# minyoungpark1/Speech-Enhancement

Hardware: AMD Instinct MI355X
Metric: utterances/sec (2 s @16 kHz) CMGAN train step (higher is better)
Workload: dtype f32 (f16x3 split); 1 GPU; cmgan generator+discriminator train step (main_gan.py train_gan loop body), batch 16/GPU, 2 s @ 16 kHz, n_fft=400 hop=100, AdamW lr 5e-4, PESQ labels supplied, kaiming-init weights; fp32 results throughout: conv and token GEMMs as scaled fp16 hi/lo splits (3 MFMAs per product, 2^-24 relative, fp32 accumulate), attention on the same scaled fp16 splits (scales from measured operand maxima), everythi; global_batch=16, parallelism=dp1

## Files before the change

### include/se_hip.h

```cpp
#ifndef SE_HIP_H
#define SE_HIP_H
#include <stddef.h>
#include <stdint.h>

#ifdef __cplusplus
extern "C" {
#endif

#define SE_MAX_TAPS 16

enum { SE_PRO_NONE = 0, SE_PRO_LN = 1, SE_PRO_SWISH = 2, SE_PRO_AFFINE_SWISH = 3,
       SE_PRO_SWISH_DROP = 4,
       SE_PRO_DROP = 5,
       SE_PRO_GATE = 6 };
enum {
  SE_EPI_BIAS = 1,
  SE_EPI_ACCUM = 2,
  SE_EPI_RESID = 4,
  SE_EPI_GLU = 8,
  SE_EPI_STATS = 16,
  SE_EPI_SWISH_GRAD = 32,
  SE_EPI_SHUFFLE2 = 64,
  SE_EPI_DROP = 128,
  SE_EPI_GLU_GATE = 2048,
// ... 118 lines not shown
                          const float* dR2, float* dX, float* dg, float* db, long M, int C, float* amax_out, void* stream);
int se_col_stats(const float* X, int ld, int x_off, double* stats, int B, long P, int C, void* stream);
int se_norm_finalize(const double* stats, const float* g, const float* beta, float* mr, float* ss,
                     int nb, int C, double count, float eps, float* running_mean, float* running_var,
                     float momentum, void* stream);
int se_bn_eval_scale(const float* rm, const float* rv, const float* g, const float* beta, float* ss,
                     float* mr, int C, float eps, void* stream);
int se_affine_prelu(const float* X, int ldx, int x_off, const float* ss, const float* slope, float* Y,
                    int ldy, int y_off, int B, long P, int C, void* stream);
int se_inorm_prelu_fwd(const float* X, int ldx, int x_off, const double* stats, const float* g, const float* beta,
                       const float* slope, float* Y, int ldy, int y_off, float* mr, int B, long P, int C, double count,
                       float eps, void* stream);
int se_inorm_prelu_fwd_amax(const float* X, int ldx, int x_off, const double* stats, const float* g, const float* beta,
                       const float* slope, float* Y, int ldy, int y_off, float* mr, int B, long P, int C, double count,
                       float eps, float* amax_out, void* stream);
int se_norm_prelu_bwd(const float* X, int ldx, int x_off, const float* mr, const float* g,
                      const float* beta, const float* slope, const float* dY, int ldy, int y_off,
                      double* red, float* dX, int lddx, int dx_off, float* dg, float* dbeta,
                      float* dslope, int B, long P, int C, int per_batch, int act, int phase, double count,
                      void* stream);
int se_norm_prelu_bwd_amax(const float* X, int ldx, int x_off, const float* mr, const float* g,
                           const float* beta, const float* slope, const float* dY, int ldy, int y_off,
                           double* red, float* dX, int lddx, int dx_off, float* dg, float* dbeta,
                           float* dslope, int B, long P, int C, int per_batch, int act, int phase, double count,
                           float* amax_out, void* stream);

int se_attn_fwd(const float* QKV, const float* E, float* O, float* LSE, int nseq, int n, int inner,
                long outer_stride, long inner_stride, long pos_stride, int maxpos, float scale, void* stream);
int se_attn_fwd_es(const float* QKV, const float* E, const void* Es, long es_plane, float* O, float* LSE, int nseq, int n,
                   int inner, long outer_stride, long inner_stride, long pos_stride, int maxpos, float scale, void* stream);
int se_attn_bwd(const float* QKV, const float* E, const float* O, const float* dO, const float* LSE,
                float* dQKV, float* dE, int nseq, int n, int inner, long outer_stride,
                long inner_stride, long pos_stride, long ntok, int maxpos, float scale, void* ws, size_t ws_bytes,
                void* stream);

int se_attn_fwd_f16(const float* QKV, const void* Es, long es_plane, const float* qkv_amax, const float* e_amax, float* O,
                    float* LSE, int nseq, int n, int inner, long outer_stride, long inner_stride, long pos_stride, int maxpos,
                    float scale, void* stream);
int se_attn_bwd_f16_phase(const float* QKV, const float* E, const float* O, const float* dO, const float* LSE,
                          const float* delta, const float* qkv_amax, const float* do_amax, float* dqkv_amax, float* dQKV, float* dE,
                          int nseq, int n, int inner, long outer_stride, long inner_stride, long pos_stride, long ntok, int maxpos,
                          float scale, void* ws, size_t ws_bytes, int phase, void* stream);

int se_dwconv31(const float* X, const float* W, const float* bias, float* Y, double* stats, int flip,
                int nseq, int n, int inner, long outer_stride, long inner_stride, long pos_stride, void* stream);
int se_dwconv31_glu_bwd(const float* dH, const float* W, const float* U, const float* G, float* dZ, float* amax_out, int nseq,
                        int n, int inner, long outer_stride, long inner_stride, long pos_stride, void* stream);
size_t se_dwconv31_wgrad_workspace_bytes(void);
int se_dwconv31_bwd_fused(const float* dH, const float* W, const float* U, const float* G, float* dZ, float* amax_out, float* dW,
                          float* dbias, float* ws, long ntok, int nseq, int n, int inner, long outer_stride, long inner_stride,
                          long pos_stride, void* stream);
int se_dwconv31_wgrad(const float* X, const float* dY, float* dW, float* dbias, int nseq, int n, int inner,
                      long outer_stride, long inner_stride, long pos_stride, float* ws, void* stream);

int se_clip_scale(const float* x, float* c, int B, int L, void* stream);
int se_reflect_pad_scale(const float* x, const float* c, float* xp, int B, int L, int pad, void* stream);
int se_reflect_pad_bwd(const float* dxp, const float* c, float* dx, int B, int L, int pad, void* stream);
int se_compress_planes(const float* R, int ldr, float* P, long rows, int F, int comp, float pre_scale, void* stream);
int se_compress_planes_bwd(const float* R, int ldr, const float* dP, float* dR, long rows, int F, int comp,
                           float pre_scale, void* stream);
int se_uncompress_rows(const float* P, float* A, int lda, long rows, int F, int comp, float post_scale, void* stream);
int se_uncompress_rows_bwd(const float* P, const float* dA, int lda, float* dP, long rows, int F, int comp,
                           float post_scale, void* stream);
int se_stft_fused(const float* x, const float* c, const float* Wf, float* P, int B, int L, int n_fft, int hop, int comp,
                  float pre_scale, void* stream);
int se_istft_fused(const float* P, const float* Wi, const float* env, float* y, int B, int T, int n_fft, int hop, int comp,
                   float post_scale, void* stream);
int se_ola(const float* Fr, const float* env, float* y, int B, int T, int n_fft, int hop, int trim, int L, void* stream);
int se_ola_bwd(const float* dy, const float* env, float* dFr, int B, int T, int n_fft, int hop, void* stream);
int se_assemble(const float* mask, int ldm, const float* nin, const float* cplx, float* est, long n, void* stream);
int se_assemble_bwd(const float* est, const float* dest, const float* nin, float* dmask, int ldm, float* dcplx,
                    long n, void* stream);
int se_mask_tail(const float* U, int ldu, const float* wb, const float* slope, float* M, long n, int F, void* stream);
int se_mask_tail_bwd(const float* U, int ldu, const float* wb, const float* slope, const float* dM, float* dU,
                     double* dwb, float* dslope, long n, int F, void* stream);
int se_glu_bwd(const float* Z, const float* dU, float* dZ, long M, int H, void* stream);
int se_glu_bwd_amax(const float* Z, const float* dU, float* dZ, long M, int H, float* amax_out, void* stream);
int se_glu_bwd_gate(const float* U, const float* G, const float* dU, float* dZ, long M, int H, float* amax_out, void* stream);
int se_gate_tanh(const float* Y, float* G, long M, int C, void* stream);
int se_gate_tanh_bwd(const float* Y, const float* dG, float* dY, long M, int C, void* stream);
int se_spec_loss(const float* A, const float* Bp, double* sums, long n, void* stream);
int se_spec_loss_bwd(const float* A, const float* Bp, float* dA, const float* up, float cmag, float cri, long n,
                     int accumulate, void* stream);
int se_l1_loss(const float* a, long lda, const float* b, long ldb, double* sums, long rows, int L, void* stream);
int se_l1_loss_bwd(const float* a, long lda, const float* b, long ldb, float* da, const float* up, float ck,
                   long rows, int L, void* stream);
int se_adamw(float* p, const float* g, float* m, float* v, long n, float lr, float b1, float b2, float eps,
             float wd, int step, void* stream);
int se_sgd_nesterov(float* p, const float* g, float* buf, long n, float lr, float momentum, int first, void* stream);
int se_dot(const float* a, const float* b, double* out, long n, void* stream);
int se_grad_clip(float* g, long n, const double* sums, int nsum, float max_norm, void* stream);
int se_lars_step(float* p, const float* g, float* mu, const long* seg_off, int nseg, long max_seg, double* norms,
                 int adapt, float lr, float wd, float momentum, float trust_coef, void* stream);
int se_lamb_step(float* p, const float* g, float* m, float* v, const long* seg_off, int nseg, long max_seg,
                 double* norms, const double* gsum, int nsum, float max_grad_norm, int adapt, int trust_clip, float lr,
                 float wd, float b1, float b2, float beta3, float eps, float bc1, float bc2, void* stream);
int se_axpbypcz(const float* a, const float* b, const float* c, float* y, float alpha, float beta, float gamma,
                long n, void* stream);

int se_spectral_norm(int n, const float* const* W, float* const* u, float* const* v, float* const* Wn, const int* h,
                     const int* w, float* sigma, int train, float eps, void* stream);
int se_spectral_norm_bwd(int n, const float* const* dWn, const float* const* Wn, const float* const* u,
                         const float* const* v, const float* sigma, float* const* dW, const int* h, const int* w, void* stream);
size_t se_disc_tail_workspace_bytes(int B);
int se_disc_tail_fwd(const float* A, int B, int P, const float* W1, const float* b1, const float* mask, const float* slope1,
                     const float* W2, const float* b2, const float* sslope, float beta, float* out, float* ws, void* stream);
// ... 38 lines not shown
```

### speech-enhancement_amd/csrc/se_dwconv.hip

```cpp
#include <type_traits>
#include "se_common.h"

struct SeqGeom {
  int nseq, n, inner;
  long outer_stride, inner_stride, pos_stride;
};
static __device__ __forceinline__ long tok_of(const SeqGeom& g, int s, int p) {
  return (long)(s / g.inner) * g.outer_stride + (long)(s % g.inner) * g.inner_stride + (long)p * g.pos_stride;
}

constexpr int DW_C = 128, DW_K = 31;
#ifdef SE_DW_NT
#define DW_STORE(p, v) __builtin_nontemporal_store((v), (p))
#else
#define DW_STORE(p, v) (*(p) = (v))
#endif
#define DW_LOAD4(p) (*reinterpret_cast<const f32x4*>(p))

struct DwArgs {
  SeqGeom g;
  const float* X; const float* W; const float* bias; float* Y; double* stats; int flip;
  const float* Z; float* amax_out; const float* U;
};

// ... 222 lines not shown
        if (i < NR) {
#pragma unroll
          for (int o = 0; o < PPS; ++o) {
            const int k = i - o;
            if (k >= 0 && k < DW_K) acc[k] = __builtin_elementwise_fma(dy[o], xg[g & 1][j], acc[k]);
          }
        }
      }
    }
  }
  float* red = xs;
  float* prow = a.part + (long)blockIdx.x * 32 * DW_C;
#pragma unroll
  for (int k0 = 0; k0 < 32; k0 += 8) {
    __syncthreads();
#pragma unroll
    for (int kk = 0; kk < 8; ++kk) {
      const int k = k0 + kk;
      const f32x2 v = k < DW_K ? acc[k < DW_K ? k : 0] : bacc;
      *reinterpret_cast<f32x2*>(&red[((ps * 8 + kk) * DW_C) + cl * 2]) = v;
    }
    __syncthreads();
    for (int i = tid; i < 8 * DW_C; i += 512) {
      int kk = i >> 7, ch = i & 127;
      float t = 0.f;
#pragma unroll
      for (int sl = 0; sl < 8; ++sl) t += red[(sl * 8 + kk) * DW_C + ch];
      prow[(k0 + kk) * DW_C + ch] = t;
    }
  }
}

__global__ void dwconv_wgrad_reduce_kernel(const float* __restrict__ part, int nwg, float* __restrict__ dW,
                                           float* __restrict__ dbias) {
  const int i = blockIdx.x * blockDim.x + threadIdx.x;
  const int per = (nwg + gridDim.y - 1) / gridDim.y, w0 = blockIdx.y * per, w1 = w0 + per < nwg ? w0 + per : nwg;
  if (i >= 32 * DW_C || w0 >= w1) return;
  float v[16];
#pragma unroll
  for (int j = 0; j < 16; ++j) v[j] = w0 + j < w1 ? part[(long)(w0 + j) * 32 * DW_C + i] : 0.f;
  float t = 0.f;
#pragma unroll
  for (int j = 0; j < 16; ++j) t += v[j];
  for (int w = w0 + 16; w < w1; ++w) t += part[(long)w * 32 * DW_C + i];
  const int k = i >> 7, ch = i & 127;
  if (k < DW_K) atomicAdd(&dW[ch * DW_K + k], t);
  else if (dbias) atomicAdd(&dbias[ch], t);
}

struct DwBwdArgs {
  SeqGeom g;
  const float* dH; const float* W; const float* U; const float* Z; float* dZ; float* amax_out; float* part;
  unsigned bytes128, bytes256;
};
constexpr int FB_PPS = 7, FB_TILE = 16 * FB_PPS, FB_ROWS = FB_TILE + DW_K - 1, FB_NLD = (FB_ROWS * 32 + 1023) / 1024,
              FB_NLU = (FB_TILE * 32 + 1023) / 1024;
typedef unsigned u32x2fb_ __attribute__((ext_vector_type(2)));
#ifndef FB_NT
#define FB_NT 8
#endif
constexpr int FB_LDS_BYTES = (FB_ROWS * DW_C + FB_TILE * DW_C + DW_K * DW_C) * 4;

__global__ __launch_bounds__(1024) void dwconv_bwd_fused_kernel(DwBwdArgs a) {
  extern __shared__ __attribute__((aligned(16))) float fb_smem[];
  float* xs = fb_smem;
  float* us = fb_smem + FB_ROWS * DW_C;
  float* wt = us + FB_TILE * DW_C;
  const int tid = threadIdx.x, cl = tid & 63, ps = __builtin_amdgcn_readfirstlane(tid >> 6);
  const unsigned cl8 = (unsigned)cl * 8u;
  const int n = a.g.n;
  for (int i = tid; i < DW_C * DW_K; i += 1024) {
    const int ch = i / DW_K, k = i - ch * DW_K;
    wt[(DW_K - 1 - k) * DW_C + ch] = a.W[i];
  }
  const __amdgpu_buffer_rsrc_t rH = make_rsrc_(a.dH, a.bytes128), rU = make_rsrc_(a.U, a.bytes128), rG = make_rsrc_(a.Z, a.bytes128),
                               rD = make_rsrc_(a.dZ, a.bytes256);
  const int tiles = (n + FB_TILE - 1) / FB_TILE;
  const long nitems = (long)a.g.nseq * tiles;
  const int xcd = blockIdx.x & 7, slot = blockIdx.x >> 3, S = gridDim.x >> 3;
  const long Q = (nitems + 7) >> 3, ibase = (long)xcd * Q, iend = ibase + Q < nitems ? ibase + Q : nitems;
  const unsigned rsb = (unsigned)(a.g.pos_stride * DW_C * 4);
  float zmax = 0.f;
  float4 ld[FB_NLD], lu[FB_NLU];
  const int lrow = tid >> 5;
  const unsigned lane_off = (unsigned)lrow * rsb + (unsigned)(tid & 31) * 16u;
  auto request_rows = [&](long it) {
    const bool live = it < iend;
    const long itc = live ? it : 0;
    const int seq = (int)(itc / tiles), p0 = (int)(itc - (long)seq * tiles) * FB_TILE;
    const unsigned base = (unsigned)(((long)(seq / a.g.inner) * a.g.outer_stride + (long)(seq % a.g.inner) * a.g.inner_stride) * (DW_C * 4));
    const int plo = 15 - p0 > 0 ? 15 - p0 : 0;
    const int phi = n - (p0 - 15) < FB_ROWS ? n - (p0 - 15) : FB_ROWS;
    const unsigned span = live && phi > plo ? (unsigned)(phi - plo) : 0u;
    const unsigned uspan = live ? (unsigned)(n - p0 < FB_TILE ? n - p0 : FB_TILE) : 0u;
#pragma unroll
    for (int k = 0; k < FB_NLD; ++k) {
      const int row = lrow + 32 * k;
      const unsigned off = base + (unsigned)(p0 - 15 + 32 * k) * rsb + lane_off;
      ld[k] = buf_load4_(rH, (unsigned)(row - plo) < span ? off : BUF_OOB_);
    }
#pragma unroll
    for (int k = 0; k < FB_NLU; ++k) {
      const int row = lrow + 32 * k;
      const unsigned off = base + (unsigned)(p0 + 32 * k) * rsb + lane_off;
      lu[k] = buf_load4_(rU, (unsigned)row < uspan ? off : BUF_OOB_);
    }
  };
  constexpr int NT = FB_NT, NGRP = 32 / NT, NPART = 16 / NGRP, PLEN = FB_TILE / NPART;
  const int tg = ps % NGRP, ph = ps / NGRP;
  f32x2 wacc[NT];
#pragma unroll
  for (int j = 0; j < NT; ++j) wacc[j] = (f32x2){0.f, 0.f};
  request_rows(ibase + slot);
  for (long it = ibase + slot; it < iend; it += S) {
    const int seq = (int)(it / tiles), p0 = (int)(it - (long)seq * tiles) * FB_TILE;
    const unsigned base = (unsigned)(((long)(seq / a.g.inner) * a.g.outer_stride + (long)(seq % a.g.inner) * a.g.inner_stride) * (DW_C * 4));
    __syncthreads();
#pragma unroll
    for (int k = 0; k < FB_NLD; ++k) {
      const int row = lrow + 32 * k;
      if (row < FB_ROWS) *reinterpret_cast<float4*>(&xs[row * DW_C + (tid & 31) * 4]) = ld[k];
    }
#pragma unroll
    for (int k = 0; k < FB_NLU; ++k) {
      const int row = lrow + 32 * k;
      if (row < FB_TILE) *reinterpret_cast<float4*>(&us[row * DW_C + (tid & 31) * 4]) = lu[k];
    }
    __syncthreads();
    const int pbase = p0 + ps * FB_PPS;
    f32x2 gt[FB_PPS];
#pragma unroll
    for (int o = 0; o < FB_PPS; ++o)
      gt[o] = __builtin_bit_cast(f32x2, buf_load2_(rG, pbase + o < n ? base + (unsigned)(pbase + o) * rsb + cl8 : BUF_OOB_));
    {
      constexpr int NR = FB_PPS + DW_K - 1;
      const float* xrow = &xs[(ps * FB_PPS) * DW_C + cl * 2];
      f32x2 acc[FB_PPS];
#pragma unroll
      for (int o = 0; o < FB_PPS; ++o) acc[o] = (f32x2){0.f, 0.f};
#pragma unroll
      for (int h = 0; h < 2; ++h) {
        constexpr int KH = 16;
        const int K0 = h * KH, K1 = h == 0 ? KH : DW_K;
        f32x2 w[KH];
#pragma unroll
        for (int k = 0; k < KH; ++k)
          if (K0 + k < K1) w[k] = *reinterpret_cast<const f32x2*>(&wt[(K0 + k) * DW_C + cl * 2]);
        const int R0 = K0, R1 = K1 - 1 + FB_PPS;
        constexpr int GA = 4;
        f32x2 xg[2][GA];
#pragma unroll
        for (int j = 0; j < GA; ++j) xg[0][j] = *reinterpret_cast<const f32x2*>(xrow + (R0 + j) * DW_C);
#pragma unroll
        for (int g = 0; g < (KH + FB_PPS - 1 + GA - 1) / GA; ++g) {
          asm volatile("" ::: "memory");
          if (R0 + (g + 1) * GA < R1) {
#pragma unroll
            for (int j = 0; j < GA; ++j)
              if (R0 + (g + 1) * GA + j < R1) xg[(g + 1) & 1][j] = *reinterpret_cast<const f32x2*>(xrow + (R0 + (g + 1) * GA + j) * DW_C);
          }
          asm volatile("" ::: "memory");
#pragma unroll
          for (int j = 0; j < GA; ++j) {
            const int i = R0 + g * GA + j;
            if (i < R1) {
#pragma unroll
              for (int o = 0; o < FB_PPS; ++o) {
                const int k = i - o;
                if (k >= K0 && k < K1) acc[o] = __builtin_elementwise_fma(xg[g & 1][j], w[k - K0], acc[o]);
              }
            }
          }
        }
      }
#pragma unroll
      for (int o = 0; o < FB_PPS; ++o) asm volatile("" : "+v"(acc[o]));
      const float* urow = &us[(ps * FB_PPS) * DW_C + cl * 2];
#pragma unroll
      for (int o = 0; o < FB_PPS; ++o) {
// ... 29 lines not shown
        constexpr int UB = 2, BOFF = 17 - NT;
        static_assert(PLEN % UB == 0, "position part not a multiple of the read group");
        f32x2 r[NT];
#pragma unroll
        for (int jj = 1; jj < NT; ++jj)
          if (!(BIAS && jj == NT - 1)) r[jj] = *reinterpret_cast<const f32x2*>(xp - jj * DW_C);
#pragma unroll 1
        for (int qq = 0; qq < PLEN; qq += UB) {
          f32x2 uu[UB], r0[UB], rb[UB];
#pragma unroll
          for (int e = 0; e < UB; ++e) {
            uu[e] = *reinterpret_cast<const f32x2*>(up + (qq + e) * DW_C);
            r0[e] = *reinterpret_cast<const f32x2*>(xp + (qq + e) * DW_C);
            if constexpr (BIAS) rb[e] = *reinterpret_cast<const f32x2*>(xp + (qq + e + BOFF) * DW_C);
          }
#pragma unroll
          for (int e = 0; e < UB; ++e) {
            r[0] = r0[e];
#pragma unroll
            for (int jj = 0; jj < NT; ++jj) {
              if (BIAS && jj == NT - 1) wacc[jj] += rb[e];
              else wacc[jj] = __builtin_elementwise_fma(uu[e], r[jj], wacc[jj]);
            }
#pragma unroll
            for (int jj = NT - 1; jj >= 1; --jj) r[jj] = r[jj - 1];
          }
        }
      };
      if (tg == NGRP - 1) phase_b(std::true_type{}); else phase_b(std::false_type{});
    }
#endif
  }
  if (a.amax_out) {
    zmax = wave_max(zmax);
    if ((tid & 63) == 0) amax_raise_(a.amax_out, zmax);
  }
  __syncthreads();
  float* red = xs;
  int t2 = threadIdx.x;
  asm volatile("" : "+v"(t2));
  const int w2 = t2 >> 6, c2 = t2 & 63;
#pragma unroll
  for (int j = 0; j < NT; ++j) *reinterpret_cast<f32x2*>(&red[((w2 / NGRP) * 32 + NT * (w2 % NGRP) + j) * DW_C + c2 * 2]) = wacc[j];
  __syncthreads();
  float* prow = a.part + (long)blockIdx.x * 32 * DW_C;
  float4 t = *reinterpret_cast<const float4*>(red + t2 * 4);
#pragma unroll
  for (int h = 1; h < NPART; ++h) {
    const float4 v = *reinterpret_cast<const float4*>(red + h * 32 * DW_C + t2 * 4);
    t = make_float4(t.x + v.x, t.y + v.y, t.z + v.z, t.w + v.w);
  }
  *reinterpret_cast<float4*>(prow + t2 * 4) = t;
}

extern "C" int se_dwconv31(const float* X, const float* W, const float* bias, float* Y, double* stats, int flip,
                           int nseq, int n, int inner, long outer_stride, long inner_stride, long pos_stride,
                           void* stream) {
  SE_REQUIRE(X && W && Y && nseq > 0 && n > 0 && inner > 0, "dwconv31: bad arguments");
  SE_REQUIRE(pos_stride > 0 && pos_stride * DW_C * 160L < (1L << 30), "dwconv31: position stride too large for 32-bit tile offsets");
  DwArgs a{{nseq, n, inner, outer_stride, inner_stride, pos_stride}, X, W, bias, Y, stats, flip, nullptr, nullptr};
  const int pps = n <= 64 ? 8 : (n <= 104 ? 13 : 14);
  const long nitems = (long)nseq * cdiv(n, 8 * pps);
  const int nblk = nitems < 512 ? (int)((nitems + 7) / 8 * 8) : 512;
#ifdef SE_DW_TWIN
  if (pps == 13) hipLaunchKernelGGL((dwconv_kernel<13, false, true>), dim3(nblk), dim3(512), 0, as_stream(stream), a);
  else if (pps == 14) hipLaunchKernelGGL((dwconv_kernel<14, false, true>), dim3(nblk), dim3(512), 0, as_stream(stream), a);
  else
#endif
  if (pps == 8) hipLaunchKernelGGL(dwconv_kernel<8>, dim3(nblk), dim3(512), 0, as_stream(stream), a);
  else if (pps == 13) hipLaunchKernelGGL(dwconv_kernel<13>, dim3(nblk), dim3(512), 0, as_stream(stream), a);
  else hipLaunchKernelGGL(dwconv_kernel<14>, dim3(nblk), dim3(512), 0, as_stream(stream), a);
  return se_check_launch("se_dwconv31");
}

extern "C" int se_dwconv31_glu_bwd(const float* dH, const float* W, const float* U, const float* G, float* dZ, float* amax_out,
                                   int nseq, int n, int inner, long outer_stride, long inner_stride, long pos_stride,
                                   void* stream) {
  SE_REQUIRE(dH && W && U && G && dZ && nseq > 0 && n > 0 && inner > 0, "dwconv31_glu_bwd: bad arguments");
  SE_REQUIRE(pos_stride > 0 && pos_stride * DW_C * 320L < (1L << 30), "dwconv31_glu_bwd: position stride too large for 32-bit tile offsets");
  DwArgs a{{nseq, n, inner, outer_stride, inner_stride, pos_stride}, dH, W, nullptr, dZ, nullptr, 1, G, amax_out, U};
  const int pps = n <= 64 ? 8 : (n <= 104 ? 13 : 14);
  const long nitems = (long)nseq * cdiv(n, 8 * pps);
  const int nblk = nitems < 512 ? (int)((nitems + 7) / 8 * 8) : 512;
#ifdef SE_DW_TWIN
  if (pps == 13) hipLaunchKernelGGL((dwconv_kernel<13, true, true>), dim3(nblk), dim3(512), 0, as_stream(stream), a);
  else if (pps == 14) hipLaunchKernelGGL((dwconv_kernel<14, true, true>), dim3(nblk), dim3(512), 0, as_stream(stream), a);
  else
#endif
  if (pps == 8) hipLaunchKernelGGL((dwconv_kernel<8, true>), dim3(nblk), dim3(512), 0, as_stream(stream), a);
  else if (pps == 13) hipLaunchKernelGGL((dwconv_kernel<13, true>), dim3(nblk), dim3(512), 0, as_stream(stream), a);
  else hipLaunchKernelGGL((dwconv_kernel<14, true>), dim3(nblk), dim3(512), 0, as_stream(stream), a);
  return se_check_launch("se_dwconv31_glu_bwd");
}

extern "C" size_t se_dwconv31_wgrad_workspace_bytes(void) { return (size_t)512 * 32 * DW_C * sizeof(float); }

extern "C" int se_dwconv31_wgrad(const float* X, const float* dY, float* dW, float* dbias, int nseq, int n,
                                 int inner, long outer_stride, long inner_stride, long pos_stride, float* ws,
                                 void* stream) {
  SE_REQUIRE(X && dY && dW && ws && nseq > 0 && n > 0 && inner > 0, "dwconv31_wgrad: bad arguments");
  SE_REQUIRE(pos_stride > 0 && pos_stride * DW_C * 160L < (1L << 30), "dwconv31_wgrad: position stride too large for 32-bit tile offsets");
  DwWgradArgs a{{nseq, n, inner, outer_stride, inner_stride, pos_stride}, X, dY, dW, dbias, ws};
  const int pps = n <= 64 ? 8 : (n <= 104 ? 13 : 14);
  const long nitems = (long)nseq * cdiv(n, 8 * pps);
  const int nblk = nitems < 512 ? (int)((nitems + 7) / 8 * 8) : 512;
  if (pps == 8) hipLaunchKernelGGL(dwconv_wgrad_kernel<8>, dim3(nblk), dim3(512), 0, as_stream(stream), a);
  else if (pps == 13) hipLaunchKernelGGL(dwconv_wgrad_kernel<13>, dim3(nblk), dim3(512), 0, as_stream(stream), a);
  else hipLaunchKernelGGL(dwconv_wgrad_kernel<14>, dim3(nblk), dim3(512), 0, as_stream(stream), a);
  hipLaunchKernelGGL(dwconv_wgrad_reduce_kernel, dim3(32 * DW_C / 256, 32), dim3(256), 0, as_stream(stream), (const float*)ws, nblk,
                     dW, dbias);
  return se_check_launch("se_dwconv31_wgrad");
}

extern "C" int se_dwconv31_bwd_fused(const float* dH, const float* W, const float* U, const float* G, float* dZ, float* amax_out,
                                     float* dW, float* dbias, float* ws, long ntok, int nseq, int n, int inner, long outer_stride,
                                     long inner_stride, long pos_stride, void* stream) {
  SE_REQUIRE(dH && W && U && G && dZ && dW && ws && nseq > 0 && n > 0 && inner > 0 && ntok > 0, "dwconv31_bwd_fused: bad arguments");
  SE_REQUIRE(ntok * (DW_C * 8L) < (1L << 32) - 4096, "dwconv31_bwd_fused: operands beyond 32-bit buffer offsets (%ld tokens)", ntok);
  SE_REQUIRE(pos_stride > 0 && (long)(nseq - 1) / inner * outer_stride + (long)(inner - 1) * inner_stride + (long)(n - 1) * pos_stride < ntok,
             "dwconv31_bwd_fused: sequence geometry reaches past %ld tokens", ntok);
  DwBwdArgs a{{nseq, n, inner, outer_stride, inner_stride, pos_stride}, dH, W, U, G, dZ, amax_out, ws,
              (unsigned)(ntok * DW_C * 4), (unsigned)(ntok * DW_C * 8)};
  const long nitems = (long)nseq * cdiv(n, FB_TILE);
  const int ncu = se_cu_count();
  int nblk = nitems < ncu ? (int)((nitems + 7) / 8 * 8) : ncu / 8 * 8;
  if (nblk > 512) nblk = 512;
  static unsigned lds_done = 0;
  SE_REQUIRE(se_raise_lds((const void*)dwconv_bwd_fused_kernel, FB_LDS_BYTES, &lds_done), "dwconv31_bwd_fused: cannot raise the LDS limit");
  hipLaunchKernelGGL(dwconv_bwd_fused_kernel, dim3(nblk), dim3(1024), FB_LDS_BYTES, as_stream(stream), a);
  hipLaunchKernelGGL(dwconv_wgrad_reduce_kernel, dim3(32 * DW_C / 256, 32), dim3(256), 0, as_stream(stream), (const float*)ws, nblk,
                     dW, dbias);
  return se_check_launch("se_dwconv31_bwd_fused");
}
```

### speech-enhancement_amd/layers.py

```python
import ctypes as C

import torch

from . import _lib as L
from . import attention as A
from . import gemm as GM
from . import ops as O

EPS = 1e-5

import os as _os
EPS = 1e-5

import os as _os
_PREC = {'f32': 0, 'bf16x3': 1, 'bf16x6': 2, 'f16x3': 3}
CONV_PRECISION = _PREC[_os.environ.get('SE_CONV_PRECISION', 'f16x3')]
ACT_SEXP = 4
PW2_F16 = True
ATTN_O_SEXP = 4
ATTN_PRECISION = [_os.environ.get('SE_ATTN_PRECISION', 'f16x3')]


WGRAD_PRECISION = [_PREC[_os.environ.get('SE_WGRAD_PRECISION', 'f16x3')]]


FUSE_LN_BWD = True
FUSE_ROWSTATS = True
FUSE_GLU_BWD = True


def set_conv_precision(name, wgrad=None):
    global CONV_PRECISION
    CONV_PRECISION = _PREC[name]
    WGRAD_PRECISION[0] = _PREC[wgrad or name]


def _conv3_shape(taps, sf, C_in, Fo=None):
    if sf != 1 or C_in < 32 or len(taps) % 3 or (Fo is not None and Fo < 2):
        return False
    for i in range(0, len(taps), 3):
        if {t[0] for t in taps[i:i + 3]} != {taps[i][0]} or sorted(abs(t[1]) for t in taps[i:i + 3]) != [0, 1, 1] or \
                {t[1] for t in taps[i:i + 3]} != {-1, 0, 1}:
            return False
    return True


def _prec(p, taps, sf, C_in, Fo=None, have_scale=True):
    if p != 3:
        return p
    return 3 if (have_scale and _conv3_shape(taps, sf, C_in, Fo)) else 2


def _prec_w(p, W, taps, sf, C_in, Fo=None, have_scale=True):
    if W.dtype == torch.float16:
        return 3
    if W.dtype == torch.bfloat16:
        return 2
    return _prec(p, taps, sf, C_in, Fo, have_scale)


class DPHooks:
    world = 1

    def allreduce(self, t):
        return t


NO_DP = DPHooks()


def _T(w):
    return w.t().contiguous()


def conv_fwd(x, B, Ti, Fi, lda, a_off, C_in, wp, bias, taps, N, To=None, Fo=None, sf=1, shuffle2=False,
             want_stats=True, a_amax=None):
    To = To or Ti
    Fo = Fo or Fi
    ep = L.EPI_BIAS | (L.EPI_STATS if want_stats else 0) | (L.EPI_SHUFFLE2 if shuffle2 else 0)
    No = N // 2 if shuffle2 else N
    d = GM.make_desc(B, To, Fo, Ti, Fi, taps, C_in, lda, N, No, a_off=a_off, sf=sf, epilogue=ep,
# ... 417 lines not shown
        mr, ss = O.norm_finalize(bnstats, g_bn, b_bn, 1, 128, count, running_mean=rm, running_var=rv, momentum=0.1)
        if buffers is not None:
            nbt = buffers.get('_nbt_pending')
            if nbt is not None:
                nbt.append(buffers[f'{p}.conv.net.5.num_batches_tracked'])
            else:
                buffers[f'{p}.conv.net.5.num_batches_tracked'] += 1
    else:
        h = O.dwconv31(u, Wdw, P[f'{p}.conv.net.4.conv.bias'], geom)
        mr, ss = O.bn_eval_scale(P[f'{p}.conv.net.5.running_mean'], P[f'{p}.conv.net.5.running_var'], g_bn, b_bn)
    sst = ss[0].t().contiguous()
    sc, sh = sst[0], sst[1]
    y3 = torch.empty(M, 64, device=x.device, dtype=torch.float32)
    bn_b = _bnd(P, ('bn', f'{p}.conv'), GM.HID_SEXP, need_k1=max(count - 1.0, 1.0) ** 0.5) if train else {}
    Wpw2 = _w(P, (f'{p}.conv.net.7.weight', 'lin'), lambda: None) if (train or 'a_amax' in bn_b) else None
    if Wpw2 is None:
        Wpw2 = P[f'{p}.conv.net.7.weight'].view(64, 128)
    st4 = torch.empty(M, 2, device=x.device, dtype=torch.float32) if FUSE_ROWSTATS else None
    GM.gemm_tap(GM.linear_desc(M, 128, 64, prologue=L.PRO_AFFINE_SWISH, epilogue=L.EPI_BIAS | L.EPI_RESID |
                               (L.EPI_ROWSTATS if FUSE_ROWSTATS else 0), alpha=1.0, ldr=64,
                               **_lin3(Wpw2, **bn_b)), h, Wpw2, y3,
                bias=P[f'{p}.conv.net.7.bias'], R=y2, ps=sc, pb=sh, AUX=st4)
    ctx['conv'] = (y2, st3, zc, u, h, mr, sc, sh, count)
    y4, ctx['ff2'] = _ff_fwd(P, f'{p}.ff2', y3, M, pf, site_seed(seed, 3), site_seed(seed, 4), st=st4)
    if FUSE_ROWSTATS:
        out, st5, ctx['out_stats'] = O.layernorm_fwd(y4, P[f'{p}.post_norm.weight'], P[f'{p}.post_norm.bias'], R=x, out_stats=True)
    else:
        out, st5 = O.layernorm_fwd(y4, P[f'{p}.post_norm.weight'], P[f'{p}.post_norm.bias'], R=x)
    ctx['post'] = (y4, st5)
    return out, ctx


def conformer_bwd(P, G, p, ctx, dout, B, T, Fq, dp=NO_DP, train=True):
    if not train:
        raise L.SeHipError('conformer_bwd in eval mode is not supported (BatchNorm uses running statistics)')
    M = dout.shape[0]
    geom = ctx['geom']
    dev = dout.device
    y4, st5 = ctx['post']
    dy4 = O.layernorm_bwd(y4, st5, P[f'{p}.post_norm.weight'], dout, G[f'{p}.post_norm.weight'],
                          G[f'{p}.post_norm.bias'], amax=_amax(dev))
    dy3 = _ff_bwd(P, G, f'{p}.ff2', ctx['ff2'], dy4, M)
    ctx['ff2'] = ctx['post'] = None
    y2, st3, zc, u, h, mr, sc, sh, count = ctx['conv']
    Wpw2 = P[f'{p}.conv.net.7.weight'].view(64, 128)
    dact = torch.empty(M, 128, device=dev, dtype=torch.float32)
    Wpw2T = _w(P, (f'{p}.conv.net.7.weight', 'T'), lambda: _T(Wpw2))
    GM.gemm_tap(GM.linear_desc(M, 64, 128, **_lin3(Wpw2T, a_amax=getattr(dy3, '_se_amax', None))), dy3, Wpw2T, dact)
    with GM.leaf_stream(h, dy3, sc, sh, getattr(dy3, '_se_amax', None)):
        GM.gemm_tap_wgrad(GM.linear_desc(M, 128, 64, prologue=L.PRO_AFFINE_SWISH,
                                         **_bnd(P, ('bn', f'{p}.conv'), GM.HID_SEXP, need_k1=max(count - 1.0, 1.0) ** 0.5),
                                         w_amax=getattr(dy3, '_se_amax', None)), h, dy3,
                          G[f'{p}.conv.net.7.weight'].view(64, 128), G[f'{p}.conv.net.7.bias'], ps=sc, pb=sh)
    dh = torch.empty(M, 128, device=dev, dtype=torch.float32)
    g_bn, b_bn = P[f'{p}.conv.net.5.weight'], P[f'{p}.conv.net.5.bias']
    if train:
        O.norm_prelu_bwd(h, 128, 0, mr, g_bn, b_bn, None, dact, 128, 0, dh, 128, 0, G[f'{p}.conv.net.5.weight'],
                         G[f'{p}.conv.net.5.bias'], None, 1, M, 128, per_batch=False, act=1,
                         allreduce=(dp.allreduce if dp.world > 1 or getattr(dp, 'force_sync', False) else None), count=count)
    else:
        raise L.SeHipError('conformer_bwd in eval mode is not supported (BatchNorm uses running statistics)')
    Wdw = P[f'{p}.conv.net.4.conv.weight'].view(128, 31)
    dw_fused = FUSE_GLU_BWD and O.DW_BWD_FUSED and M * 1024 < (1 << 32) - 4096
    if dw_fused:
        dzc = O.dwconv31_bwd_fused(dh, Wdw, u, zc, G[f'{p}.conv.net.4.conv.weight'].view(128, 31), G[f'{p}.conv.net.4.conv.bias'], geom,
                                   amax=_amax(dev))
        du = None
    elif FUSE_GLU_BWD:
        dzc = O.dwconv31_glu_bwd(dh, Wdw, u, zc, geom, amax=_amax(dev))
        du = None
    else:
        du = O.dwconv31(dh, Wdw, None, geom, flip=True)
    if not dw_fused:
        with GM.leaf_stream(u, dh):
            O.dwconv31_wgrad(u, dh, G[f'{p}.conv.net.4.conv.weight'].view(128, 31), G[f'{p}.conv.net.4.conv.bias'], geom)
    if not FUSE_GLU_BWD:
        dzc = O.glu_bwd_gate(u, zc, du, M, 128, amax=_amax(dev))
    Wpw1 = P[f'{p}.conv.net.2.weight'].view(256, 64)
    Wpw1T = _w(P, (f'{p}.conv.net.2.weight', 'T'), lambda: _T(Wpw1))
    fused_pw1 = GM.LNBWD_FUSED and FUSE_LN_BWD and Wpw1T.dtype == torch.float16 and getattr(dzc, '_se_amax', None) is not None
    if not fused_pw1:
        with GM.leaf_stream(y2, dzc, st3, dzc._se_amax):
            GM.gemm_tap_wgrad(GM.linear_desc(M, 64, 256, prologue=L.PRO_LN, w_amax=dzc._se_amax, **_bnd(P, ('ln', f'{p}.conv'), GM.LN_SEXP)), y2, dzc,
                              G[f'{p}.conv.net.2.weight'].view(256, 64),
                              G[f'{p}.conv.net.2.bias'], rowstats=st3, ps=P[f'{p}.conv.net.0.weight'],
                              pb=P[f'{p}.conv.net.0.bias'])
    if fused_pw1:
        dy2 = GM.gemm_ln_bwd_wgrad(dzc, Wpw1T, y2, st3, P[f'{p}.conv.net.0.weight'], P[f'{p}.conv.net.0.bias'], dy3,
                                   G[f'{p}.conv.net.0.weight'], G[f'{p}.conv.net.0.bias'], G[f'{p}.conv.net.2.weight'].view(256, 64),
                                   G[f'{p}.conv.net.2.bias'], out_amax=_amax(dev), in_bound=_bnd(P, ('ln', f'{p}.conv'), 0).get('a_amax'))
    elif FUSE_LN_BWD and GM.LINEAR_PRECISION in (2, 3):
        dy2 = GM.gemm_ln_bwd(dzc, Wpw1T, y2, st3, P[f'{p}.conv.net.0.weight'], dy3, G[f'{p}.conv.net.0.weight'],
                             G[f'{p}.conv.net.0.bias'], out_amax=_amax(dev))
    else:
        dl3 = torch.empty(M, 64, device=dev, dtype=torch.float32)
        GM.gemm_tap(GM.linear_desc(M, 256, 64, **_lin3(Wpw1T, a_amax=dzc._se_amax)), dzc, Wpw1T, dl3)
        dy2 = O.layernorm_bwd(y2, st3, P[f'{p}.conv.net.0.weight'], dl3, G[f'{p}.conv.net.0.weight'],
                              G[f'{p}.conv.net.0.bias'], dR=dy3, amax=_amax(dev))
        del dl3
    ctx['conv'] = None
    del dact, dh, du, dzc, dy3, dy4
    y1, st2, Wqkv, qkv, o, lse, maxpos, pa, sa, qkv_amax = ctx['attn']
    Wo = P[f'{p}.attn.fn.to_out.weight']
    do = torch.empty(M, 64, device=dev, dtype=torch.float32)
    WoT = _w(P, (f'{p}.attn.fn.to_out.weight', 'T'), lambda: _T(Wo))
    do_amax = O.zeros(1, device=dev) if qkv_amax is not None else None
    delta = torch.empty(M, 4, device=dev, dtype=torch.float32) if (qkv_amax is not None and A.f16_shape_ok(geom, maxpos)) else None
    GM.gemm_tap(GM.linear_desc(M, 64, 64, prologue=L.PRO_DROP if pa > 0 else L.PRO_NONE, pro_seed=sa, drop_p=pa, y_amax=do_amax,
                               epilogue=L.EPI_DELTA if delta is not None else 0, ldr=64 if delta is not None else 0,
                               **_lin3(WoT, a_amax=getattr(dy2, '_se_amax', None))), dy2, WoT, do, R=o if delta is not None else None, AUX=delta)
    with GM.leaf_stream(o, dy2, getattr(dy2, '_se_amax', None), qkv_amax):
        GM.gemm_tap_wgrad(GM.linear_desc(M, 64, 64, epilogue=L.EPI_DROP if pa > 0 else 0, epi_seed=sa, drop_p=pa,
                                         w_amax=getattr(dy2, '_se_amax', None),
                                         **(dict(a_amax=qkv_amax) if qkv_amax is not None else dict(a_sexp=ATTN_O_SEXP))), o, dy2,
                          G[f'{p}.attn.fn.to_out.weight'], G[f'{p}.attn.fn.to_out.bias'])
    dqkv = A.attn_bwd(qkv, P[f'{p}.attn.fn.rel_pos_emb.weight'], o, do, lse, geom,
                      G[f'{p}.attn.fn.rel_pos_emb.weight'], maxpos=maxpos, scale=0.25,
# ... 214 lines not shown
```

### speech-enhancement_amd/ops.py

```python
import ctypes as C
import os as _os

import torch

from . import _lib as L

f32 = torch.float32
f64 = torch.float64
_i, _l, _f, _d = C.c_int, C.c_long, C.c_float, C.c_double


def _new(*shape, like, dtype=f32):
    return torch.empty(*shape, device=like.device, dtype=dtype)


class ZeroArena:

    def __init__(self):
        self.buf, self.off, self.high, self.active, self.missed = None, 0, 0, False, 0

    def begin(self, device, min_bytes=16 << 20):
        need = max(min_bytes, 2 * (self.high + self.missed))
        if self.buf is None or self.buf.device != device or self.buf.numel() < need:
            self.buf = torch.zeros(need, device=device, dtype=torch.uint8)
# ... 100 lines not shown


def norm_prelu_bwd(x, ldx, x_off, mr, g, beta, slope, dy, ldy, y_off, dx, lddx, dx_off, dg, dbeta, dslope, B, P, C_,
                   per_batch=True, act=0, allreduce=None, count=None, amax=None):
    if count is None:
        count = float(P if per_batch else P * B)
    red = zeros(L.lib().se_norm_prelu_bwd_workspace_bytes(_i(B), _i(C_), _i(int(per_batch))) // 8, device=x.device, dtype=f64)
    args = lambda phase: (L.ptr(x), _i(ldx), _i(x_off), L.ptr(mr), L.ptr(g), L.ptr(beta), L.ptr(slope),
                          L.ptr(dy), _i(ldy), _i(y_off), L.ptr(red), L.ptr(dx), _i(lddx), _i(dx_off), L.ptr(dg),
                          L.ptr(dbeta), L.ptr(dslope), _i(B), _l(P), _i(C_), _i(int(per_batch)), _i(act),
                          _i(phase), _d(count), L.ptr(amax), L.stream())
    if allreduce is None:
        L.call('se_norm_prelu_bwd_amax', *args(1 | 2 | 8 | 16))
    else:
        L.call('se_norm_prelu_bwd_amax', *args(1 | 4 | 16))
        allreduce(red)
        L.call('se_norm_prelu_bwd_amax', *args(2))
    return dx


def dwconv31(x, w, bias, geom, stats=None, flip=False):
    y = torch.empty_like(x)
    nseq, n, inner, os_, is_, ps = geom
    L.call('se_dwconv31', L.ptr(x), L.ptr(w), L.ptr(bias), L.ptr(y), L.ptr(stats), _i(int(flip)), _i(nseq), _i(n),
           _i(inner), _l(os_), _l(is_), _l(ps), L.stream(), _key='dwconv31 (fwd / dgrad)', _bytes=8.0 * x.numel())
    return y


def dwconv31_glu_bwd(dh, w, u, gate, geom, amax=None):
    M = dh.shape[0]
    dz = torch.empty(M, 256, device=dh.device, dtype=torch.float32)
    nseq, n, inner, os_, is_, ps = geom
    L.call('se_dwconv31_glu_bwd', L.ptr(dh), L.ptr(w), L.ptr(u), L.ptr(gate), L.ptr(dz), L.ptr(amax), _i(nseq), _i(n), _i(inner), _l(os_),
           _l(is_), _l(ps), L.stream(), _key='dwconv31 dgrad + glu_bwd', _bytes=4.0 * (3 * dh.numel() + dz.numel()))
    dz._se_amax = amax
    return dz


DW_BWD_FUSED = _os.environ.get('SE_DW_BWD_FUSED', '1') != '0'


def dwconv31_bwd_fused(dh, w, u, gate, dw, dbias, geom, amax=None):
    M = dh.shape[0]
    dz = torch.empty(M, 256, device=dh.device, dtype=torch.float32)
    nseq, n, inner, os_, is_, ps = geom
    ws = _new(L.lib().se_dwconv31_wgrad_workspace_bytes() // 4, like=dh)
    L.call('se_dwconv31_bwd_fused', L.ptr(dh), L.ptr(w), L.ptr(u), L.ptr(gate), L.ptr(dz), L.ptr(amax), L.ptr(dw), L.ptr(dbias),
           L.ptr(ws), _l(M), _i(nseq), _i(n), _i(inner), _l(os_), _l(is_), _l(ps), L.stream(),
           _key='dwconv31 dgrad + glu_bwd + wgrad', _bytes=4.0 * (3 * dh.numel() + dz.numel()))
    dz._se_amax = amax
    return dz


def dwconv31_wgrad(x, dy, dw, dbias, geom):
    nseq, n, inner, os_, is_, ps = geom
    ws = _new(L.lib().se_dwconv31_wgrad_workspace_bytes() // 4, like=x)
    L.call('se_dwconv31_wgrad', L.ptr(x), L.ptr(dy), L.ptr(dw), L.ptr(dbias), _i(nseq), _i(n), _i(inner), _l(os_),
           _l(is_), _l(ps), L.ptr(ws), L.stream(), _key='dwconv31_wgrad (+ reduce)', _bytes=8.0 * x.numel())


COMP = {None: 0, 'none': 0, 'norm': 0, 'pow': 1, 'log': 2}


def clip_scale(x):
    B, L_ = x.shape
    c = _new(B, like=x)
    L.call('se_clip_scale', L.ptr(x), L.ptr(c), _i(B), _i(L_), L.stream())
    return c


def reflect_pad_scale(x, c, pad):
    B, L_ = x.shape
    xp = _new(B, L_ + 2 * pad, like=x)
    L.call('se_reflect_pad_scale', L.ptr(x), L.ptr(c), L.ptr(xp), _i(B), _i(L_), _i(pad), L.stream())
    return xp


def compress_planes(R, ldr, rows, F_, comp, pre_scale=1.0):
    P = _new(rows, F_, 4, like=R)
    L.call('se_compress_planes', L.ptr(R), _i(ldr), L.ptr(P), _l(rows), _i(F_), _i(COMP[comp]), _f(pre_scale),
           L.stream())
    return P


def uncompress_rows(P, rows, F_, lda, comp, post_scale=1.0):
    A = _zeros(rows, lda, like=P)
    L.call('se_uncompress_rows', L.ptr(P), L.ptr(A), _i(lda), _l(rows), _i(F_), _i(COMP[comp]), _f(post_scale),
           L.stream())
    return A


def uncompress_rows_bwd(P, dA, lda, dP, rows, F_, comp, post_scale=1.0):
    L.call('se_uncompress_rows_bwd', L.ptr(P), L.ptr(dA), _i(lda), L.ptr(dP), _l(rows), _i(F_), _i(COMP[comp]),
           _f(post_scale), L.stream())
    return dP


def ola(frames, env, B, T, n_fft, hop, trim=None, L_out=None):
    trim = n_fft // 2 if trim is None else trim
    L_out = hop * (T - 1) if L_out is None else L_out
    y = _new(B, L_out, like=frames)
    L.call('se_ola', L.ptr(frames), L.ptr(env), L.ptr(y), _i(B), _i(T), _i(n_fft), _i(hop), _i(trim), _i(L_out),
           L.stream())
    return y


# ... 114 lines not shown
```

Baseline: 290.9 utterances/sec.

## Fold BatchNorm+swish backward apply into fused depthwise-conv backward kernel

Splits the BatchNorm/swish backward into a reduction-only pass that produces per-channel sums, and applies the per-element BN/swish gradient inside the fused depthwise conv31 backward kernel while it loads rows. This avoids writing and re-reading the full dh tensor and drops one elementwise pass over the conv activations. In exchange the fused kernel also loads the pre-BN activations, uses more LDS and registers, and runs with a smaller weight-gradient group size. dgamma/dbeta are accumulated by block 0 when there is no allreduce.

```diff
diff --git a/include/se_hip.h b/include/se_hip.h
--- a/include/se_hip.h
+++ b/include/se_hip.h
@@ -194,6 +194,10 @@
                           long pos_stride, void* stream);
 int se_dwconv31_wgrad(const float* X, const float* dY, float* dW, float* dbias, int nseq, int n, int inner,
                       long outer_stride, long inner_stride, long pos_stride, float* ws, void* stream);
+int se_dwconv31_bn_bwd_fused(const float* dY, const float* H, const float* mr, const float* gamma, const float* beta, const double* red,
+                             double count, float* dgamma, float* dbeta, const float* W, const float* U, const float* G, float* dZ,
+                             float* amax_out, float* dW, float* dbias, float* ws, long ntok, int nseq, int n, int inner,
+                             long outer_stride, long inner_stride, long pos_stride, void* stream);
 
 int se_clip_scale(const float* x, float* c, int B, int L, void* stream);
 int se_reflect_pad_scale(const float* x, const float* c, float* xp, int B, int L, int pad, void* stream);
diff --git a/speech-enhancement_amd/csrc/se_dwconv.hip b/speech-enhancement_amd/csrc/se_dwconv.hip
--- a/speech-enhancement_amd/csrc/se_dwconv.hip
+++ b/speech-enhancement_amd/csrc/se_dwconv.hip
@@ -298,6 +298,7 @@
   SeqGeom g;
   const float* dH; const float* W; const float* U; const float* Z; float* dZ; float* amax_out; float* part;
   unsigned bytes128, bytes256;
+  const float* X; const float* mr; const float* gamma; const float* beta; const double* red; double count; float* dgamma; float* dbeta;
 };
 constexpr int FB_PPS = 7, FB_TILE = 16 * FB_PPS, FB_ROWS = FB_TILE + DW_K - 1, FB_NLD = (FB_ROWS * 32 + 1023) / 1024,
               FB_NLU = (FB_TILE * 32 + 1023) / 1024;
@@ -305,13 +306,19 @@
 #ifndef FB_NT
 #define FB_NT 8
 #endif
+#ifndef FB_NT_BN
+#define FB_NT_BN 4
+#endif
 constexpr int FB_LDS_BYTES = (FB_ROWS * DW_C + FB_TILE * DW_C + DW_K * DW_C) * 4;
-
-__global__ __launch_bounds__(1024) void dwconv_bwd_fused_kernel(DwBwdArgs a) {
+constexpr int FB_LDS_BYTES_BN = FB_LDS_BYTES + 7 * DW_C * 4;
+
+template <bool BN>
+static __device__ __forceinline__ void dwconv_bwd_fused_body(const DwBwdArgs& a) {
   extern __shared__ __attribute__((aligned(16))) float fb_smem[];
   float* xs = fb_smem;
   float* us = fb_smem + FB_ROWS * DW_C;
   float* wt = us + FB_TILE * DW_C;
+  float* bnt = wt + DW_K * DW_C;
   const int tid = threadIdx.x, cl = tid & 63, ps = __builtin_amdgcn_readfirstlane(tid >> 6);
   const unsigned cl8 = (unsigned)cl * 8u;
   const int n = a.g.n;
@@ -319,15 +326,32 @@
     const int ch = i / DW_K, k = i - ch * DW_K;
     wt[(DW_K - 1 - k) * DW_C + ch] = a.W[i];
   }
+  if constexpr (BN) {
+    if (tid < DW_C) {
+      const int c = tid;
+      const float mean = a.mr[2 * c], rstd = a.mr[2 * c + 1];
+      bnt[c] = mean;
+      bnt[DW_C + c] = rstd;
+      bnt[2 * DW_C + c] = rstd * a.gamma[c];
+      bnt[3 * DW_C + c] = (float)(a.red[c * 3] / a.count);
+      bnt[4 * DW_C + c] = (float)(a.red[c * 3 + 1] / a.count);
+      bnt[5 * DW_C + c] = a.gamma[c];
+      bnt[6 * DW_C + c] = a.beta[c];
+      if (a.dgamma && blockIdx.x == 0) {
+        a.dgamma[c] += (float)a.red[c * 3 + 1];
+        a.dbeta[c] += (float)a.red[c * 3];
+      }
+    }
+  }
   const __amdgpu_buffer_rsrc_t rH = make_rsrc_(a.dH, a.bytes128), rU = make_rsrc_(a.U, a.bytes128), rG = make_rsrc_(a.Z, a.bytes128),
-                               rD = make_rsrc_(a.dZ, a.bytes256);
+                               rD = make_rsrc_(a.dZ, a.bytes256), rX = make_rsrc_(BN ? a.X : a.dH, a.bytes128);
   const int tiles = (n + FB_TILE - 1) / FB_TILE;
   const long nitems = (long)a.g.nseq * tiles;
   const int xcd = blockIdx.x & 7, slot = blockIdx.x >> 3, S = gridDim.x >> 3;
   const long Q = (nitems + 7) >> 3, ibase = (long)xcd * Q, iend = ibase + Q < nitems ? ibase + Q : nitems;
   const unsigned rsb = (unsigned)(a.g.pos_stride * DW_C * 4);
   float zmax = 0.f;
-  float4 ld[FB_NLD], lu[FB_NLU];
+  float4 ld[FB_NLD], lu[FB_NLU], lh[BN ? FB_NLD : 1];
   const int lrow = tid >> 5;
   const unsigned lane_off = (unsigned)lrow * rsb + (unsigned)(tid & 31) * 16u;
   auto request_rows = [&](long it) {
@@ -344,6 +368,7 @@
       const int row = lrow + 32 * k;
       const unsigned off = base + (unsigned)(p0 - 15 + 32 * k) * rsb + lane_off;
       ld[k] = buf_load4_(rH, (unsigned)(row - plo) < span ? off : BUF_OOB_);
+      if constexpr (BN) lh[BN ? k : 0] = buf_load4_(rX, (unsigned)(row - plo) < span ? off : BUF_OOB_);
     }
 #pragma unroll
     for (int k = 0; k < FB_NLU; ++k) {
@@ -352,7 +377,7 @@
       lu[k] = buf_load4_(rU, (unsigned)row < uspan ? off : BUF_OOB_);
     }
   };
-  constexpr int NT = FB_NT, NGRP = 32 / NT, NPART = 16 / NGRP, PLEN = FB_TILE / NPART;
+  constexpr int NT = BN ? FB_NT_BN : FB_NT, NGRP = 32 / NT, NPART = 16 / NGRP, PLEN = FB_TILE / NPART;
   const int tg = ps % NGRP, ph = ps / NGRP;
   f32x2 wacc[NT];
 #pragma unroll
@@ -362,15 +387,49 @@
     const int seq = (int)(it / tiles), p0 = (int)(it - (long)seq * tiles) * FB_TILE;
     const unsigned base = (unsigned)(((long)(seq / a.g.inner) * a.g.outer_stride + (long)(seq % a.g.inner) * a.g.inner_stride) * (DW_C * 4));
     __syncthreads();
-#pragma unroll
-    for (int k = 0; k < FB_NLD; ++k) {
-      const int row = lrow + 32 * k;
-      if (row < FB_ROWS) *reinterpret_cast<float4*>(&xs[row * DW_C + (tid & 31) * 4]) = ld[k];
-    }
-#pragma unroll
-    for (int k = 0; k < FB_NLU; ++k) {
-      const int row = lrow + 32 * k;
-      if (row < FB_TILE) *reinterpret_cast<float4*>(&us[row * DW_C + (tid & 31) * 4]) = lu[k];
+    if constexpr (BN) {
+#pragma unroll
+      for (int k = 0; k < FB_NLU; ++k) {
+        const int row = lrow + 32 * k;
+        if (row < FB_TILE) *reinterpret_cast<float4*>(&us[row * DW_C + (tid & 31) * 4]) = lu[k];
+      }
+      const int c4 = (tid & 31) * 4;
+      const int plo = 15 - p0 > 0 ? 15 - p0 : 0;
+      const int phi = n - (p0 - 15) < FB_ROWS ? n - (p0 - 15) : FB_ROWS;
+      const unsigned span = phi > plo ? (unsigned)(phi - plo) : 0u;
+#pragma unroll
+      for (int j = 0; j < 4; ++j) {
+        const float mean = bnt[c4 + j], rstd = bnt[DW_C + c4 + j], ag = bnt[2 * DW_C + c4 + j], m1 = bnt[3 * DW_C + c4 + j];
+        const float m2 = bnt[4 * DW_C + c4 + j], gg = bnt[5 * DW_C + c4 + j], bt = bnt[6 * DW_C + c4 + j];
+#pragma unroll
+        for (int k = 0; k < FB_NLD; ++k) {
+          const bool real = (unsigned)(lrow + 32 * k - plo) < span;
+          float& d = j == 0 ? ld[k].x : (j == 1 ? ld[k].y : (j == 2 ? ld[k].z : ld[k].w));
+          const float h = j == 0 ? lh[k].x : (j == 1 ? lh[k].y : (j == 2 ? lh[k].z : lh[k].w));
+          const float xh = (h - mean) * rstd;
+          const float u = xh * gg + bt;
+          const float du = d * swish_gradf_(u);
+          d = real ? ag * (du - m1 - xh * m2) : 0.f;
+        }
+      }
+#pragma unroll
+      for (int k = 0; k < FB_NLD; ++k) {
+        const int row = lrow + 32 * k;
+        if (row < FB_ROWS) *reinterpret_cast<float4*>(&xs[row * DW_C + c4]) = ld[k];
+      }
+    } else {
+#pragma unroll
+      for (int k = 0; k < FB_NLD; ++k) {
+        const int row = lrow + 32 * k;
+        if (row < FB_ROWS) *reinterpret_cast<float4*>(&xs[row * DW_C + (tid & 31) * 4]) = ld[k];
+      }
+    }
+    if constexpr (!BN) {
+#pragma unroll
+      for (int k = 0; k < FB_NLU; ++k) {
+        const int row = lrow + 32 * k;
+        if (row < FB_TILE) *reinterpret_cast<float4*>(&us[row * DW_C + (tid & 31) * 4]) = lu[k];
+      }
     }
     __syncthreads();
     const int pbase = p0 + ps * FB_PPS;
@@ -506,6 +565,9 @@
   }
   *reinterpret_cast<float4*>(prow + t2 * 4) = t;
 }
+
+__global__ __launch_bounds__(1024) void dwconv_bwd_fused_kernel(DwBwdArgs a) { dwconv_bwd_fused_body<false>(a); }
+__global__ __launch_bounds__(1024) void dwconv_bwd_fused_kernel_bn(DwBwdArgs a) { dwconv_bwd_fused_body<true>(a); }
 
 extern "C" int se_dwconv31(const float* X, const float* W, const float* bias, float* Y, double* stats, int flip,
                            int nseq, int n, int inner, long outer_stride, long inner_stride, long pos_stride,
@@ -586,3 +648,26 @@
                      dW, dbias);
   return se_check_launch("se_dwconv31_bwd_fused");
 }
+
+extern "C" int se_dwconv31_bn_bwd_fused(const float* dY, const float* H, const float* mr, const float* gamma, const float* beta, const double* red,
+                                        double count, float* dgamma, float* dbeta, const float* W, const float* U, const float* G, float* dZ,
+                                        float* amax_out, float* dW, float* dbias, float* ws, long ntok, int nseq, int n, int inner,
+                                        long outer_stride, long inner_stride, long pos_stride, void* stream) {
+  SE_REQUIRE(dY && H && mr && gamma && beta && red && count > 0 && (!dgamma == !dbeta) && W && U && G && dZ && dW && ws && nseq > 0 && n > 0 &&
+             inner > 0 && ntok > 0, "dwconv31_bn_bwd_fused: bad arguments");
+  SE_REQUIRE(ntok * (DW_C * 8L) < (1L << 32) - 4096, "dwconv31_bn_bwd_fused: operands beyond 32-bit buffer offsets (%ld tokens)", ntok);
+  SE_REQUIRE(pos_stride > 0 && (long)(nseq - 1) / inner * outer_stride + (long)(inner - 1) * inner_stride + (long)(n - 1) * pos_stride < ntok,
+             "dwconv31_bn_bwd_fused: sequence geometry reaches past %ld tokens", ntok);
+  DwBwdArgs a{{nseq, n, inner, outer_stride, inner_stride, pos_stride}, dY, W, U, G, dZ, amax_out, ws,
+              (unsigned)(ntok * DW_C * 4), (unsigned)(ntok * DW_C * 8), H, mr, gamma, beta, red, count, dgamma, dbeta};
+  const long nitems = (long)nseq * cdiv(n, FB_TILE);
+  const int ncu = se_cu_count();
+  int nblk = nitems < ncu ? (int)((nitems + 7) / 8 * 8) : ncu / 8 * 8;
+  if (nblk > 512) nblk = 512;
+  static unsigned lds_done = 0;
+  SE_REQUIRE(se_raise_lds((const void*)dwconv_bwd_fused_kernel_bn, FB_LDS_BYTES_BN, &lds_done), "dwconv31_bn_bwd_fused: cannot raise the LDS limit");
+  hipLaunchKernelGGL(dwconv_bwd_fused_kernel_bn, dim3(nblk), dim3(1024), FB_LDS_BYTES_BN, as_stream(stream), a);
+  hipLaunchKernelGGL(dwconv_wgrad_reduce_kernel, dim3(32 * DW_C / 256, 32), dim3(256), 0, as_stream(stream), (const float*)ws, nblk,
+                     dW, dbias);
+  return se_check_launch("se_dwconv31_bn_bwd_fused");
+}
diff --git a/speech-enhancement_amd/layers.py b/speech-enhancement_amd/layers.py
--- a/speech-enhancement_amd/layers.py
+++ b/speech-enhancement_amd/layers.py
@@ -27,6 +27,7 @@
 FUSE_LN_BWD = True
 FUSE_ROWSTATS = True
 FUSE_GLU_BWD = True
+FUSE_BN_BWD = True
 
 
 def set_conv_precision(name, wgrad=None):
@@ -550,17 +551,22 @@
                                          **_bnd(P, ('bn', f'{p}.conv'), GM.HID_SEXP, need_k1=max(count - 1.0, 1.0) ** 0.5),
                                          w_amax=getattr(dy3, '_se_amax', None)), h, dy3,
                           G[f'{p}.conv.net.7.weight'].view(64, 128), G[f'{p}.conv.net.7.bias'], ps=sc, pb=sh)
-    dh = torch.empty(M, 128, device=dev, dtype=torch.float32)
     g_bn, b_bn = P[f'{p}.conv.net.5.weight'], P[f'{p}.conv.net.5.bias']
-    if train:
-        O.norm_prelu_bwd(h, 128, 0, mr, g_bn, b_bn, None, dact, 128, 0, dh, 128, 0, G[f'{p}.conv.net.5.weight'],
-                         G[f'{p}.conv.net.5.bias'], None, 1, M, 128, per_batch=False, act=1,
-                         allreduce=(dp.allreduce if dp.world > 1 or getattr(dp, 'force_sync', False) else None), count=count)
-    else:
-        raise L.SeHipError('conformer_bwd in eval mode is not supported (BatchNorm uses running statistics)')
     Wdw = P[f'{p}.conv.net.4.conv.weight'].view(128, 31)
     dw_fused = FUSE_GLU_BWD and O.DW_BWD_FUSED and M * 1024 < (1 << 32) - 4096
-    if dw_fused:
+    allreduce = dp.allreduce if dp.world > 1 or getattr(dp, 'force_sync', False) else None
+    bn_fold = FUSE_BN_BWD and dw_fused
+    if not bn_fold:
+        dh = torch.empty(M, 128, device=dev, dtype=torch.float32)
+        O.norm_prelu_bwd(h, 128, 0, mr, g_bn, b_bn, None, dact, 128, 0, dh, 128, 0, G[f'{p}.conv.net.5.weight'],
+                         G[f'{p}.conv.net.5.bias'], None, 1, M, 128, per_batch=False, act=1, allreduce=allreduce, count=count)
+    if bn_fold:
+        red = O.bn_swish_bwd_sums(h, mr, g_bn, b_bn, dact, G[f'{p}.conv.net.5.weight'], G[f'{p}.conv.net.5.bias'], count, allreduce=allreduce)
+        dzc = O.dwconv31_bn_bwd_fused(dact, h, mr, g_bn, b_bn, red, count, Wdw, u, zc, G[f'{p}.conv.net.4.conv.weight'].view(128, 31),
+                                      G[f'{p}.conv.net.4.conv.bias'], geom, amax=_amax(dev),
+                                      **({} if allreduce is not None else dict(dg=G[f'{p}.conv.net.5.weight'], dbeta=G[f'{p}.conv.net.5.bias'])))
+        dh = du = None
+    elif dw_fused:
         dzc = O.dwconv31_bwd_fused(dh, Wdw, u, zc, G[f'{p}.conv.net.4.conv.weight'].view(128, 31), G[f'{p}.conv.net.4.conv.bias'], geom,
                                    amax=_amax(dev))
         du = None
diff --git a/speech-enhancement_amd/ops.py b/speech-enhancement_amd/ops.py
--- a/speech-enhancement_amd/ops.py
+++ b/speech-enhancement_amd/ops.py
@@ -176,6 +176,30 @@
     return dz
 
 
+def bn_swish_bwd_sums(h, mr, g, beta, dy, dg, dbeta, count, allreduce=None):
+    M = h.shape[0]
+    red = zeros(L.lib().se_norm_prelu_bwd_workspace_bytes(_i(1), _i(128), _i(0)) // 8, device=h.device, dtype=f64)
+    L.call('se_norm_prelu_bwd_amax', L.ptr(h), _i(128), _i(0), L.ptr(mr), L.ptr(g), L.ptr(beta), L.ptr(None), L.ptr(dy), _i(128), _i(0),
+           L.ptr(red), L.ptr(dy), _i(128), _i(0), L.ptr(dg), L.ptr(dbeta), L.ptr(None), _i(1), _l(M), _i(128), _i(0), _i(1),
+           _i(1 | 16 | (4 if allreduce is not None else 0)), _d(count), L.ptr(None), L.stream())
+    if allreduce is not None:
+        allreduce(red)
+    return red
+
+
+def dwconv31_bn_bwd_fused(dy, h, mr, gamma, beta, red, count, w, u, gate, dw, dbias, geom, dg=None, dbeta=None, amax=None):
+    M = dy.shape[0]
+    dz = torch.empty(M, 256, device=dy.device, dtype=torch.float32)
+    nseq, n, inner, os_, is_, ps = geom
+    ws = _new(L.lib().se_dwconv31_wgrad_workspace_bytes() // 4, like=dy)
+    L.call('se_dwconv31_bn_bwd_fused', L.ptr(dy), L.ptr(h), L.ptr(mr), L.ptr(gamma), L.ptr(beta), L.ptr(red), _d(count), L.ptr(dg),
+           L.ptr(dbeta), L.ptr(w), L.ptr(u), L.ptr(gate), L.ptr(dz), L.ptr(amax), L.ptr(dw), L.ptr(dbias), L.ptr(ws), _l(M), _i(nseq),
+           _i(n), _i(inner), _l(os_), _l(is_), _l(ps), L.stream(), _key='dwconv31 bn_bwd + dgrad + glu_bwd + wgrad',
+           _bytes=4.0 * (4 * dy.numel() + dz.numel()))
+    dz._se_amax = amax
+    return dz
+
+
 def dwconv31_wgrad(x, dy, dw, dbias, geom):
     nseq, n, inner, os_, is_, ps = geom
     ws = _new(L.lib().se_dwconv31_wgrad_workspace_bytes() // 4, like=x)
```

Result: faster. 297.6 utterances/sec, median of 6 (+2.3%).
